# pierluigiferrari/lane_tracker

Hardware: AMD Instinct MI355X
Metric: frames/sec at 1280x720 (end-to-end hot path: undistort+warp+filter_lane_points+sliding_window_search+fit_poly) (higher is better)
Workload: dtype u8; 1 GPU; BASELINE config 3: batch of 256 synthetic lane-like 1280x720 frames per GPU, HBM-resident; warp+filter_lane_points chain + sliding_window_search (26 levels) + fit_poly; bev=1080x1100, parallelism=frames sharded x1, one process per GPU, collective=none (single process), gathered_records_checked=0, streams_per_gpu=4

## Files before the change

include/lane_tracker_amd.h:

```cpp
#ifndef LANE_TRACKER_AMD_H
#define LANE_TRACKER_AMD_H
#include <stddef.h>
#include <stdint.h>

#ifdef __cplusplus
extern "C" {
#endif
#pragma GCC visibility push(default)

#define LT_ABI_VERSION 5

typedef enum lt_status {
    LT_OK = 0,
    LT_ERR_INVALID = -1,
    LT_ERR_HIP = -2,
    LT_ERR_NOMEM = -3,
    LT_ERR_CAPACITY = -4,
    LT_ERR_STATE = -5
} lt_status;

typedef struct lt_ctx lt_ctx;

typedef struct lt_calib {
    int32_t img_w, img_h;
// ... 270 lines not shown
int  lt_calib_warp_table(const lt_calib* calib, int16_t* xy, uint16_t* frac);
int  lt_calib_undistort_table(const lt_calib* calib, int row0, int row1, int16_t* xy, uint16_t* frac);
int  lt_calib_lab_tables(uint16_t* gamma256, uint16_t* cbrt3072, int32_t* coeffs9);
int  lt_calib_ellipse(int k, int32_t* halfwidths , int* taps);

typedef struct lt_gather lt_gather;
int  lt_gather_init(lt_ctx* ctx, int rank, int world, const char* id_path, int timeout_s, lt_gather** out);
int  lt_gather_world(lt_gather* g, int* rank, int* world);
int  lt_gather_reserve(lt_gather* g, int records_per_rank);
int  lt_gather_stage(lt_gather* g, int first_slot, int n, int at);
int  lt_gather_records(lt_gather* g, int n_records, lt_lane_record* out_host);
int  lt_gather_host(lt_gather* g, const void* in, size_t bytes, void* out);
int  lt_gather_barrier(lt_gather* g);
void lt_gather_destroy(lt_gather* g);

int  lt_timer_start(lt_ctx* ctx);
int  lt_timer_stop(lt_ctx* ctx, float* ms);
int  lt_set_stage_timing(lt_ctx* ctx, int enabled);
int  lt_stage_reset(lt_ctx* ctx);
int  lt_stage_ms(lt_ctx* ctx, float* ms, int32_t* launches, int n);
const char* lt_stage_name(int stage);
#define LT_NO_CONTEXT (-2147483647 - 1)
int  lt_last_threshold_path(lt_ctx* ctx);
int  lt_last_tophat_path(lt_ctx* ctx);
int  lt_tophat_split_form(int h, int w, int k, int nbands);
int  lt_last_adaptive_path(lt_ctx* ctx);
int  lt_last_overlay_launches(lt_ctx* ctx);

#pragma GCC visibility pop
#ifdef __cplusplus
}
#endif
#endif
```

lane_tracker_amd/_native.py:

```python
import ctypes as C
import math
import os
import subprocess
import weakref

import numpy as np

_HERE = os.path.dirname(os.path.abspath(__file__))
LIB_PATH = os.environ.get("LANE_TRACKER_AMD_LIB") or os.path.join(_HERE, "liblane_tracker_amd.so")
NUM_STAGES = 12
ABI_VERSION = 5

PLANE_R, PLANE_LAB_B, PLANE_TOPHAT_R, PLANE_TOPHAT_B, PLANE_MERGED, PLANE_MASK = range(6)


class NativeError(RuntimeError):
    pass


class Calib(C.Structure):
    _fields_ = [("img_w", C.c_int32), ("img_h", C.c_int32), ("warp_w", C.c_int32), ("warp_h", C.c_int32),
                ("cam_matrix", C.c_double * 9), ("dist_coeffs", C.c_double * 5), ("M", C.c_double * 9)]


# ... 167 lines not shown
    "lt_calib_lab_tables": (C.c_int, [_P, _P, _P]),
    "lt_calib_ellipse": (C.c_int, [C.c_int, _P, C.POINTER(C.c_int)]),
    "lt_gather_init": (C.c_int, [_P, C.c_int, C.c_int, C.c_char_p, C.c_int, C.POINTER(_P)]),
    "lt_gather_world": (C.c_int, [_P, C.POINTER(C.c_int), C.POINTER(C.c_int)]),
    "lt_gather_reserve": (C.c_int, [_P, C.c_int]),
    "lt_gather_stage": (C.c_int, [_P, C.c_int, C.c_int, C.c_int]),
    "lt_gather_records": (C.c_int, [_P, C.c_int, _P]),
    "lt_gather_host": (C.c_int, [_P, _P, C.c_size_t, _P]),
    "lt_gather_barrier": (C.c_int, [_P]),
    "lt_gather_destroy": (None, [_P]),
    "lt_timer_start": (C.c_int, [_P]),
    "lt_timer_stop": (C.c_int, [_P, C.POINTER(C.c_float)]),
    "lt_set_stage_timing": (C.c_int, [_P, C.c_int]),
    "lt_stage_reset": (C.c_int, [_P]),
    "lt_stage_ms": (C.c_int, [_P, C.POINTER(C.c_float), C.POINTER(C.c_int32), C.c_int]),
    "lt_stage_name": (C.c_char_p, [C.c_int]),
    "lt_device_cache_trim": (C.c_int, [C.c_size_t]),
    "lt_device_cache_stats": (C.c_int, [C.POINTER(C.c_size_t), C.POINTER(C.c_size_t), C.POINTER(C.c_size_t), C.POINTER(C.c_int)]),
    "lt_device_cache_counters": (C.c_int, [C.POINTER(C.c_ulonglong)] * 4),
    "lt_host_memory_stats": (C.c_int, [C.POINTER(C.c_size_t)] * 3),
    "lt_set_download_method": (C.c_int, [_P, C.c_int]),
    "lt_download_stats": (C.c_int, [_P, _P, _P, _P, _P, _P]),
    "lt_last_threshold_path": (C.c_int, [_P]),
    "lt_last_tophat_path": (C.c_int, [_P]),
    "lt_tophat_split_form": (C.c_int, [C.c_int, C.c_int, C.c_int, C.c_int]),
    "lt_last_adaptive_path": (C.c_int, [_P]),
    "lt_set_input_format": (C.c_int, [_P, C.c_int, _P]),
    "lt_get_input_format": (C.c_int, [_P, C.POINTER(C.c_int), _P]),
    "lt_set_input_size": (C.c_int, [_P, C.c_int, C.c_int]),
    "lt_get_input_size": (C.c_int, [_P, C.POINTER(C.c_int), C.POINTER(C.c_int)]),
    "lt_get_input_rows": (C.c_int, [_P, C.POINTER(C.c_int), C.POINTER(C.c_int)]),
    "lt_yuv_to_rgb": (C.c_int, [_P, _P, C.c_int, C.c_int, C.c_int, _P, _P]),
    "lt_bayer_to_rgb": (C.c_int, [_P, _P, C.c_int, C.c_int, C.c_int, _P]),
    "lt_set_raw_lut": (C.c_int, [_P, _P]),
    "lt_get_raw_lut": (C.c_int, [_P, _P, C.POINTER(C.c_int)]),
    "lt_set_raw_lut_wide": (C.c_int, [_P, _P, C.c_size_t]),
    "lt_get_raw_lut_wide": (C.c_int, [_P, _P, C.c_size_t]),
    "lt_raw16_to_rgb": (C.c_int, [_P, _P, C.c_int, C.c_int, C.c_int, _P, _P]),
    "lt_set_raw_color": (C.c_int, [_P, _P, _P, C.c_int]),
    "lt_get_raw_color": (C.c_int, [_P, _P, _P, C.POINTER(C.c_int)]),
    "lt_raw_to_rgb_color": (C.c_int, [_P, _P, C.c_int, C.c_int, C.c_int, _P, C.c_size_t, _P, _P, _P]),
    "lt_set_raw_shading": (C.c_int, [_P, _P, C.c_int, C.c_int, _P, C.c_int]),
    "lt_get_raw_shading": (C.c_int, [_P, _P, C.POINTER(C.c_int), C.POINTER(C.c_int), _P, C.POINTER(C.c_int)]),
    "lt_get_raw_shading_plane": (C.c_int, [_P, _P]),
    "lt_raw_to_rgb_shaded": (C.c_int, [_P, _P, C.c_int, C.c_int, C.c_int, _P, C.c_size_t, _P, _P, _P, C.c_int, C.c_int, _P, _P]),
    "lt_attach_device_frames": (C.c_int, [_P, _P, C.c_int, C.c_int]),
# ... 1290 lines not shown
        coef = (C.c_double * 3)()
        bad = C.c_int(0)
        _check(self.lib.lt_fit_poly2(self._h, ys.ctypes.data, xs.ctypes.data, int(ys.size), self.warp_h, self.warp_w,
                                     coef, C.byref(bad)))
        if bad.value:
            from .lane_tracker import _minimum_norm_parabola
            return _minimum_norm_parabola(ys, xs)
        return np.array(coef[:], np.float64)

    def timer_start(self):
        _check(self.lib.lt_timer_start(self._h))

    def timer_stop(self):
        ms = C.c_float(0)
        _check(self.lib.lt_timer_stop(self._h, C.byref(ms)))
        return ms.value

    def set_stage_timing(self, enabled):
        _check(self.lib.lt_set_stage_timing(self._h, int(bool(enabled))))

    def last_threshold_path(self):
        return int(self.lib.lt_last_threshold_path(self._h))

    def last_tophat_path(self):
        return int(self.lib.lt_last_tophat_path(self._h))

    def last_adaptive_path(self):
        return int(self.lib.lt_last_adaptive_path(self._h))

    def stage_reset(self):
        _check(self.lib.lt_stage_reset(self._h))

    def stage_ms(self):
        ms = (C.c_float * NUM_STAGES)()
        ln = (C.c_int32 * NUM_STAGES)()
        _check(self.lib.lt_stage_ms(self._h, ms, ln, NUM_STAGES))
        return {self.lib.lt_stage_name(i).decode(): (ms[i], ln[i]) for i in range(NUM_STAGES)}


class Gather:

    def __init__(self, ctx, rank, world, id_path, timeout_s=120):
        self._g = None
        self.ctx, self.lib = ctx, ctx.lib
        g = _P()
        _check(self.lib.lt_gather_init(ctx._h, int(rank), int(world), os.fsencode(id_path), int(timeout_s), C.byref(g)))
# ... 49 lines not shown
```

lane_tracker_amd/csrc/lt_api.cpp:

```cpp
#include <algorithm>
#include <atomic>
#include <cmath>
#include <cstdarg>
#include <cstdio>
#include <cstdlib>
#include <chrono>
#include <condition_variable>
#include <cstring>
#include <deque>
#include <map>
#include <memory>
#include <mutex>
#include <string>
#include <thread>
#include <tuple>
#include <vector>
#include <immintrin.h>
#include <sys/mman.h>
#include <unistd.h>

#include <hip/hip_ext.h>

#include "bayer_arith.h"
#include "front_arith.h"
// ... 231 lines not shown

int ensure_band_sums(lt_ctx* c, int nbands) {
    if (nbands <= c->maxbands) return LT_OK;
    int rc = sync_all(c);
    if (rc) return rc;
    dev_free(c->d_band_sums);
    if ((rc = dev_alloc(&c->d_band_sums, (size_t)c->capacity * nbands * c->calib.warp_w))) return rc;
    c->maxbands = nbands;
    return LT_OK;
}

static void preload_kernels(int device, hipStream_t s) {
    static std::mutex m;
    static std::vector<int> done;
    std::lock_guard<std::mutex> g(m);
    if (std::find(done.begin(), done.end(), device) != done.end()) return;
    done.push_back(device);
    TraceScope ts_("lt_create:preload_kernels");
    preload_k_frontend(s);
    preload_k_filter(s);
    preload_k_tophat(s);
    preload_k_threshold(s);
    preload_k_threshold_walk(s);
    preload_k_adaptive_walk(s);
    preload_k_search(s);
    preload_k_overlay(s);
    preload_k_search_viz(s);
    (void)hipStreamSynchronize(s);
    (void)hipGetLastError();
}

int ensure_bev(lt_ctx* c) {
    if (c->d_bev) return LT_OK;
    return dev_alloc(&c->d_bev, (size_t)c->capacity * c->bev_bytes);
}

void mark_masks(lt_ctx* c, int first, int n, int bits_ok, int u8_ok) {
    for (int i = first; i < first + n && i < (int)c->mask_bits_ok.size(); ++i) {
        c->mask_bits_ok[(size_t)i] = (uint8_t)bits_ok;
        c->mask_u8_ok[(size_t)i] = (uint8_t)u8_ok;
    }
}
bool masks_have_bits(const lt_ctx* c, int first, int n) {
    for (int i = first; i < first + n; ++i)
        if (!c->mask_bits_ok[(size_t)i]) return false;
    return true;
}
static int ensure_mask_plane(lt_ctx* c) {
    if (c->masks.d_plane[P_MASK]) return LT_OK;
    const int rc = c->masks.ensure_plane(P_MASK);
    if (rc) return rc;
    HIP_TRY(hipMemsetAsync(c->masks.d_plane[P_MASK], 0, (size_t)c->capacity * c->masks.plane_bytes, c->stream));
    HIP_TRY(hipStreamSynchronize(c->stream));
    return LT_OK;
}
static ChainEnv chain_env(lt_ctx* c) {
    return ChainEnv{&c->se29, &c->se55, c->brute_tophat, c->walk_min_pixels, &c->streams, c->stage_timing ? c : nullptr,
                    &c->last_threshold_path, &c->last_adaptive_path, &c->last_tophat_path};
}
int ensure_u8_masks(lt_ctx* c, int first, int n) {
    bool any = false;
    for (int i = first; i < first + n; ++i) any = any || !c->mask_u8_ok[(size_t)i];
    int rc = ensure_mask_plane(c);
    if (rc) return rc;
    if (!any) return LT_OK;
    if ((rc = sync_all(c))) return rc;
    for (int i = first; i < first + n;) {
        if (c->mask_u8_ok[(size_t)i]) { ++i; continue; }
        int j = i;
        while (j < first + n && !c->mask_u8_ok[(size_t)j]) ++j;
        launch_bits_to_u8(c->stream, slot_bits(c, i, true).bits, slot_mask(c, i),
                          c->calib.warp_h, c->calib.warp_w, c->masks.plane_bytes, c->masks.bits_stride, j - i);
        for (int k = i; k < j; ++k) c->mask_u8_ok[(size_t)k] = 1;
        i = j;
    }
    HIP_TRY(hipGetLastError());
    HIP_TRY(hipStreamSynchronize(c->stream));
    return LT_OK;
}

int make_search_geom(lt_ctx* c, const lt_search_params* p, bool band, SearchGeom& g) {
// ... 2578 lines not shown
}

int lt_timer_start(lt_ctx* c) {
    if (!c) return fail(LT_ERR_INVALID, "null context");
    { int rc = sync_all(c); if (rc) return rc; }
    HIP_TRY(hipEventRecord(c->ev0, c->stream));
    return LT_OK;
}

int lt_timer_stop(lt_ctx* c, float* ms) {
    if (!c || !ms) return fail(LT_ERR_INVALID, "null argument");
    { int rc = sync_all(c); if (rc) return rc; }
    HIP_TRY(hipEventRecord(c->ev1, c->stream));
    HIP_TRY(hipEventSynchronize(c->ev1));
    HIP_TRY(hipEventElapsedTime(ms, c->ev0, c->ev1));
    return LT_OK;
}

int lt_last_threshold_path(lt_ctx* c) {
    if (!c) { (void)fail(LT_ERR_INVALID, "null context"); return LT_NO_CONTEXT; }
    return c->last_threshold_path;
}

int lt_last_tophat_path(lt_ctx* c) {
    if (!c) { (void)fail(LT_ERR_INVALID, "null context"); return LT_NO_CONTEXT; }
    return c->last_tophat_path;
}

int lt_last_overlay_launches(lt_ctx* c) {
    if (!c) { (void)fail(LT_ERR_INVALID, "null context"); return LT_NO_CONTEXT; }
    return c->last_overlay_launches;
}

int lt_tophat_split_form(int h, int w, int k, int nbands) {
    if (h <= 0 || w <= 0 || nbands <= 0) return 0;
    const int band_rows = (h + nbands - 1) / nbands;
    return lt::tophat_split_form(h, w, k, band_rows, (h + band_rows - 1) / band_rows, (w & 3) == 0 && w >= 4) ? 1 : 0;
}

int lt_last_adaptive_path(lt_ctx* c) {
    if (!c) { (void)fail(LT_ERR_INVALID, "null context"); return LT_NO_CONTEXT; }
    return c->last_adaptive_path;
}

int lt_set_stage_timing(lt_ctx* c, int enabled) {
    if (!c) return fail(LT_ERR_INVALID, "null context");
// ... 44 lines not shown
```

lane_tracker_amd/csrc/lt_ctx.h:

```cpp
#pragma once
#include <hip/hip_runtime.h>

#include <algorithm>
#include <functional>
#include <memory>
#include <vector>

#include "lt_internal.h"

namespace lt {

int fail(int code, const char* fmt, ...) __attribute__((format(printf, 2, 3)));

#define HIP_TRY(expr)                                                                               \
    do {                                                                                            \
        hipError_t e_ = (expr);                                                                     \
        if (e_ != hipSuccess) return lt::fail(LT_ERR_HIP, "%s failed: %s", #expr, hipGetErrorString(e_)); \
    } while (0)

enum Stage {
    ST_UNDISTORT = 0, ST_WARP_SPLIT, ST_ERODE_R, ST_TOPHAT_R, ST_ERODE_B, ST_TOPHAT_B, ST_THRESHOLD, ST_MERGE,
    ST_OPEN, ST_SWS_FIT, ST_BAND_FIT, ST_SPLIT_BEV
};

// ... 105 lines not shown
    uint32_t* d_raw_cc = nullptr;
    size_t raw_cc_bytes = 0;
    bool raw_shade_set = false;
    std::vector<uint16_t> raw_mesh;
    int raw_mesh_w = 0, raw_mesh_h = 0;
    lt::RawShade raw_shade = {};
    uint16_t* d_raw_gain = nullptr;
    int src_w = 0, src_h = 0;
    uint8_t* d_src = nullptr;
    size_t src_bytes = 0, src_stride = 0;
    uint32_t* d_rs_xt = nullptr;
    int32_t* d_rs_yt = nullptr;
    std::vector<int32_t> rs_yt;
    lt::SurfEntry* d_surf = nullptr;
    std::vector<lt::SurfEntry> surf;
    std::vector<uint8_t> attached;
    std::vector<uint8_t> drawn;
    uint32_t* d_und = nullptr;
    size_t und_px = 0;
    lt::MaskArena masks;
    lt::VizRing viz;
    int last_threshold_path = -1;
    int last_tophat_path = -1;
    int last_adaptive_path = -1;
    long long walk_min_pixels = 80LL * 1100 * 1080;
    std::vector<uint8_t> mask_bits_ok, mask_u8_ok;
    std::vector<uint8_t> frame_full, annot_full;
    std::vector<uint8_t> front_ok;
    lt_lane_record* d_rec = nullptr;
    double* d_prev = nullptr;
    uint32_t* d_pix = nullptr;
    int32_t* d_cent = nullptr;
    uint32_t* d_band_sums = nullptr;
    lt_search_item* d_items = nullptr;
    lt_search_item* h_items = nullptr;
    int items_cap = 0;
    hipEvent_t items_ev = nullptr;
    int maxpix = 0, maxlev = 0, maxbands = 0;
    bool have_mask = false;
    bool brute_tophat = false;
    int16_t* d_oxy = nullptr;
    uint16_t* d_ofrac = nullptr;
    bool have_overlay = false;
    int16_t* d_spans = nullptr;
    uint8_t* d_annot = nullptr;
    uint8_t* d_strip = nullptr;
// ... 322 lines not shown
            }
        }
        if (c->ev_used + 2 > c->ev_pool.size()) return;
        a = c->ev_pool[c->ev_used++];
        b = c->ev_pool[c->ev_used++];
        (void)hipEventRecord(a, st);
    }
    ~StageScope() {
        if (!a) return;
        (void)hipEventRecord(b, st);
        c->pending.push_back({stage, a, b});
    }
};

int validate_filter(const lt_filter_params* p);
struct ChainEnv {
    const EllipseSE *se29 = nullptr, *se55 = nullptr;
    bool brute_tophat = false;
    long long walk_min_pixels = 0;
    const std::vector<hipStream_t>* streams = nullptr;
    lt_ctx* timing = nullptr;
    int *threshold_path = nullptr, *adaptive_path = nullptr;
    int* tophat_path = nullptr;
};
int run_mask_chain(MaskArena& a, const ChainEnv& env, hipStream_t s, int first, int n, const lt_filter_params* p, int h, int w,
                   int call_frames, bool u8_mask = false);

}
```

lane_tracker_amd/csrc/lt_internal.h:

```cpp
#pragma once
#include <hip/hip_runtime.h>
#include <stdint.h>

#include <vector>

#include <cstdlib>

#include "../../include/lane_tracker_amd.h"
#include "yuv_arith.h"

#ifdef LT_EXPERIMENTS
#define LT_EXP_ENV(name) std::getenv(name)
#else
#define LT_EXP_ENV(name) (static_cast<const char*>(nullptr))
#endif

namespace lt {

struct RemapTable {
    std::vector<int16_t> xy;
    std::vector<uint16_t> frac;
    int rows = 0, cols = 0;
};
void build_warp_table(const lt_calib& c, RemapTable& t);
// ... 90 lines not shown
    const uint16_t* ofrac;
};
static_assert(sizeof(OvTables) == 16, "OvTables: 16 bytes, one scalar load");
struct OvSets {
    const OvTables* sets = nullptr;
    const uint8_t* ids = nullptr;
};
int launch_inplace(hipStream_t s, int layout, const SurfEntry* tab, const SurfEntry* entries, int n, int h, int w, const int rows4[4],
                   InplaceLane l, InplaceText t, YuvCoef kin, const int32_t* rgb2yuv, OvSets per_slot = OvSets());
int launch_draw_to_surfaces(hipStream_t s, int layout, const uint8_t* rgb, size_t rgb_stride, int h, int w, const SurfEntry* entries,
                            int n, const OvTables* sets, const uint8_t* ids, InplaceLane l, InplaceText t, int lane_r0, int lane_r1,
                            const int32_t* coeffs);
void launch_split_bev(hipStream_t s, const uint8_t* bev, size_t bev_stride, int npix, const uint16_t* gamma_tab,
                      const uint16_t* cbrt_tab, const int32_t* coeffs, uint8_t* planeR, uint8_t* planeB,
                      size_t plane_stride, int n);
void launch_undistorted_to_rgb(hipStream_t s, const uint32_t* und, size_t und_px, int first_slot, int nrows, int w, uint8_t* out,
                               int n);

void preload_k_frontend(hipStream_t s);
void preload_k_filter(hipStream_t s);
void preload_k_tophat(hipStream_t s);
void preload_k_threshold(hipStream_t s);
void preload_k_threshold_walk(hipStream_t s);
void preload_k_adaptive_walk(hipStream_t s);
void preload_k_search(hipStream_t s);
void preload_k_overlay(hipStream_t s);

bool launch_overlay_lane_strip(hipStream_t s, const uint8_t* frames, size_t frame_stride, uint8_t* strips, size_t strip_stride,
                               const int16_t* oxy, const uint16_t* ofrac, const int16_t* spans, size_t span_stride_rows, int img_w,
                               int row0, int row1, int bh, int bw, float alpha, int n);
int launch_overlay_lane(hipStream_t s, const uint8_t* frames, uint8_t* out, size_t frame_stride, const int16_t* oxy,
                        const uint16_t* ofrac, const int16_t* spans, size_t span_stride_rows, int img_h, int img_w,
                        int bh, int bw, float alpha, int n, const int* rows4 = nullptr, OvSets per_slot = OvSets());
constexpr int LT_SPAN_ARG_ROWS = 1104;
void launch_store_word(hipStream_t s, unsigned* dev_word, unsigned value);
bool lane_spans_from_regions_available(int bh, int n_rows);
bool launch_lane_spans_from_regions(hipStream_t s, const double* ploty, const double* ploty2, int n_rows, int bh, int bw, int16_t* spans, int n);
bool launch_lane_spans_from_fit(hipStream_t s, const lt_lane_record* rec, const double* prev_sum, int count, const double* ploty,
                                const double* ploty2, int n_rows, int bh, int bw, int16_t* spans);
bool launch_overlay_lane_one(hipStream_t s, const uint8_t* frame, uint8_t* out, const int16_t* oxy, const uint16_t* ofrac,
                             const int16_t* spans_host, int img_h, int img_w, int bh, int bw, float alpha, const int* rows4);
void launch_overlay_text(hipStream_t s, uint8_t* out, size_t frame_stride, int img_h, int img_w, const uint8_t* atlas,
                         const uint8_t* advance, int first_char, int n_glyphs, int gw, int gh, const uint8_t* lines,
                         const int16_t* xpos, int nl, int len, int slot_chars, int y0, int step, int n);
void launch_copy_from_pinned(hipStream_t s, void* dst, const void* src_pinned, size_t bytes);
bool launch_copy_to_pinned(hipStream_t s, void* dst_pinned, const void* src, size_t bytes);
// ... 29 lines not shown
                          unsigned long long* bits_v = nullptr);
void launch_pack_merge(hipStream_t s, const uint8_t* tr, const uint8_t* tb, const uint8_t* labb, const uint8_t* nb,
                       int noise_thresh, int use_noise, unsigned long long* bits, int h, int w, size_t plane_stride,
                       size_t bits_stride, int n);
void launch_open5_bits(hipStream_t s, const unsigned long long* merged, unsigned long long* eroded, uint8_t* mask, int h,
                       int w, size_t plane_stride, size_t bits_stride, int n);
struct MergeInputs {
    unsigned long long* dst = nullptr;
    const unsigned long long* more[3] = {nullptr, nullptr, nullptr};
    int n_more = 0;
    const unsigned long long *and0 = nullptr, *and1 = nullptr;
};
inline int merge_planes(const MergeInputs& in) {
    if (!in.dst || (in.n_more != 0 && in.n_more != 1 && in.n_more != 3)) return 0;
    for (int i = 0; i < 3; ++i)
        if ((in.more[i] != nullptr) != (i < in.n_more)) return 0;
    if ((in.and0 != nullptr) != (in.and1 != nullptr) || (in.and0 && in.n_more != 3)) return 0;
    return in.and0 ? 6 : in.n_more + 1;
}
bool bilateral_walk_supported(int k_r, int C_r, int k_b, int C_b, int h, int w, int pitch, size_t plane_stride);
int launch_bilateral_walk(hipStream_t s, const uint8_t* thr, int k_r, int C_r, const uint8_t* thb, int k_b, int C_b,
                          unsigned long long* merged, unsigned long long* s1, unsigned long long* s2, unsigned long long* s3,
                          int h, int w, int pitch, size_t plane_stride, size_t bits_stride, int n);
void launch_or4_bits(hipStream_t s, const MergeInputs& in, int h, int w, size_t bits_stride, int n);
bool noise_walk_supported(int k_n, int C_n, int h, int w, int pitch, size_t plane_stride);
int launch_noise_walk(hipStream_t s, const uint8_t* braw, int k_n, int C_n, int noise_thresh, unsigned long long* noise_h,
                      unsigned long long* noise_v, int h, int w, int pitch, size_t plane_stride, size_t bits_stride, int n);
bool launch_merge_open5(hipStream_t s, const MergeInputs& in, unsigned long long* opened, int h, int w, size_t bits_stride, int n);
bool launch_or_open5_small(hipStream_t s, const MergeInputs& in, unsigned long long* opened, int h, int w, size_t bits_stride, int n);
void launch_open5_to_bits(hipStream_t s, const unsigned long long* merged, unsigned long long* eroded,
                          unsigned long long* opened, int h, int w, size_t bits_stride, int n);
void launch_bits_to_u8(hipStream_t s, const unsigned long long* bits, uint8_t* out, int h, int w, size_t plane_stride,
                       size_t bits_stride, int n);


struct SearchGeom {
    int h, w;
    int ww, wh, hw;
    int img_height;
    int img_center, y_start, nlevels, limit;
    int nbands;
    int ignore_sides, search_range, def_left, def_right;
    int band_top, band_bottom;
    double mu, bandwidth;
    int maxpix, maxlev;
};
// ... 67 lines not shown
```

lane_tracker_amd/csrc/lt_mask_chain.cpp:

```cpp
#include "lt_ctx.h"

namespace lt {

int validate_filter(const lt_filter_params* p) {
    if (!p) return fail(LT_ERR_INVALID, "null filter params");
    if (p->filter_type != 0 && p->filter_type != 1)
        return fail(LT_ERR_INVALID, "Unexpected filter mode. Expected modes are 'bilateral' or 'neighborhood'.");
    if (p->ksize_r < 1 || p->ksize_b < 1 || (p->mask_noise && p->ksize_noise < 1))
        return fail(LT_ERR_INVALID, "filter sizes must be >= 1");
    if (p->filter_type == 1 && ((p->ksize_r & 1) == 0 || (p->ksize_b & 1) == 0))
        return fail(LT_ERR_INVALID, "'neighborhood' block sizes must be odd (cv2.adaptiveThreshold requirement)");
    if (p->ksize_r > 128 || p->ksize_b > 128 || p->ksize_noise > 128)
        return fail(LT_ERR_INVALID, "filter size too large (max 128)");
    return LT_OK;
}

namespace {

enum TophatForm {
    TH_NONE,
    TH_BRUTE,
    TH_PAIR,
    TH_BATCH
};
// ... 5 lines not shown
    const lt_filter_params* p;
    const int first, n, h, w;
    const bool u8_mask;
    const size_t ps = a.plane_bytes, off = (size_t)first * ps;
    uint8_t *R = a.d_plane[P_R] + off, *B = a.d_plane[P_B] + off, *thR = a.d_plane[P_THR] + off, *thB = a.d_plane[P_THB] + off, *t0 = a.d_plane[P_T0] + off;
    unsigned long long *mbits = a.d_bits_merged + (size_t)first * a.bits_stride, *ebits = a.d_bits_eroded + (size_t)first * a.bits_stride;
    bool walk = false;
    int tophat_path = 0;
    uint8_t *thRd = thR, *thBd = thB, *bpad = nullptr;
    int dpitch = 0;

    int scratch(int idx, uint8_t*& q) {
        const int rc = a.ensure_plane(idx);
        if (!rc) q = a.d_plane[idx] + off;
        return rc;
    }

    int choose_walk(int call_frames) {
        walk = p->filter_type == 0 && !env.brute_tophat && a.walk_planes() && (long long)call_frames * h * w >= env.walk_min_pixels &&
               bilateral_walk_supported(p->ksize_r, p->C_r, p->ksize_b, p->C_b, h, w, a.th_pitch, a.th_pad_bytes) &&
               (!p->mask_noise || noise_walk_supported(p->ksize_noise, p->C_noise, h, w, a.th_pitch, a.th_pad_bytes));
        if (p->filter_type != 0) return LT_OK;
        if (env.threshold_path) *env.threshold_path = walk ? 1 : 0;
        for (int i = first; i < first + n && i < (int)a.th_padded.size(); ++i) a.th_padded[(size_t)i] = walk ? 1 : 0;
        if (!walk) return LT_OK;
        dpitch = a.th_pitch;
        thRd = a.d_th_pad[0] + (size_t)first * a.th_pad_bytes;
        thBd = a.d_th_pad[1] + (size_t)first * a.th_pad_bytes;
        if (p->mask_noise) {
            const int rc = a.ensure_noise_buffers();
            if (rc) return rc;
            bpad = a.d_b_pad + (size_t)first * a.th_pad_bytes;
        }
        return LT_OK;
    }

    int tophat_b(const MorphZone& zone, int* form) {
        if (bpad && launch_morph_runs(s, t0, thBd, B, h, w, 55, true, ps, n, dpitch, a.th_pad_bytes, bpad, zone, form)) return LT_OK;
        launch_morph_runs(s, t0, thBd, B, h, w, 55, true, ps, n, dpitch, a.th_pad_bytes, nullptr, zone, form);
        if (bpad)
            for (int i = 0; i < n; ++i)
                HIP_TRY(hipMemcpy2DAsync(bpad + (size_t)i * a.th_pad_bytes, (size_t)a.th_pitch, B + (size_t)i * ps, (size_t)w, (size_t)w,
                                         (size_t)h, hipMemcpyDeviceToDevice, s));
        return LT_OK;
    }

// ... 31 lines not shown
                zone.stride_dwords = a.zone_stride;
            }
            int f29e = 0, f29d = 0, f55e = 0, f55d = 0;
            { StageScope t(tm, ST_ERODE_R, s);  launch_morph_runs(s, R, t0, nullptr, h, w, 29, false, ps, n, 0, 0, nullptr, zone, &f29e); }
            { StageScope t(tm, ST_TOPHAT_R, s); launch_morph_runs(s, t0, thRd, R, h, w, 29, true, ps, n, dpitch, a.th_pad_bytes, nullptr, zone, &f29d); }
            { StageScope t(tm, ST_ERODE_B, s);  launch_morph_runs(s, B, t0, nullptr, h, w, 55, false, ps, n, 0, 0, nullptr, zone, &f55e); }
            { StageScope t(tm, ST_TOPHAT_B, s); const int rc = tophat_b(zone, &f55d); if (rc) return rc; }
            tophat_path = (f29e && f29d ? 1 : 0) | (f55e && f55d ? 2 : 0);
        }
        if (env.tophat_path && p->filter_type == 0) *env.tophat_path = tophat_path;
        return LT_OK;
    }

    int thresholds(TophatForm form, MergeInputs& in) {
        const size_t bs = a.bits_stride;
        const int noise = p->mask_noise ? 1 : 0;
        in = MergeInputs{};
        in.dst = mbits;
        uint8_t *t1 = nullptr, *t2 = nullptr;
        if (p->filter_type == 0) {
            StageScope t(env.timing, ST_THRESHOLD, s);
            if (walk) {
                unsigned long long *tbits = a.d_bits_tmp + (size_t)first * bs, *ubits = a.d_bits_tmp2 + (size_t)first * bs;
                if (launch_bilateral_walk(s, thRd, p->ksize_r, p->C_r, thBd, p->ksize_b, p->C_b, mbits, ebits, tbits, ubits, h, w, a.th_pitch,
                                          a.th_pad_bytes, bs, n))
                    return fail(LT_ERR_STATE, "the bilateral walk refused parameters its own predicate accepted");
                in.more[0] = ebits, in.more[1] = tbits, in.more[2] = ubits, in.n_more = 3;
                if (!noise) return LT_OK;
                unsigned long long *n1 = a.d_bits_n1 + (size_t)first * bs, *n2 = a.d_bits_n2 + (size_t)first * bs;
                if (launch_noise_walk(s, bpad, p->ksize_noise, p->C_noise, p->noise_thresh, n1, n2, h, w, a.th_pitch, a.th_pad_bytes, bs, n))
                    return fail(LT_ERR_STATE, "the greenery-mask walk refused parameters its own predicate accepted");
                in.and0 = n1; in.and1 = n2;
                return LT_OK;
            }
            if (form == TH_PAIR && !noise &&
                launch_bilateral_bits(s, thR, p->ksize_r, p->C_r, thB, p->ksize_b, p->C_b, B, p->ksize_noise, p->C_noise, p->noise_thresh, 0,
                                      mbits, h, w, ps, bs, n, ebits) == 0) {
                in.more[0] = ebits, in.n_more = 1;
                return LT_OK;
            }
            if (launch_bilateral_bits(s, thR, p->ksize_r, p->C_r, thB, p->ksize_b, p->C_b, B, p->ksize_noise, p->C_noise, p->noise_thresh, noise,
                                      mbits, h, w, ps, bs, n) == 0)
                return LT_OK;
            { int rc = scratch(P_T1, t1); if (!rc) rc = scratch(P_T2, t2); if (rc) return rc; }
            launch_bilateral(s, thR, t1, h, w, p->ksize_r, p->C_r, 0, 255, 0, ps, n);
            launch_bilateral(s, thB, t2, h, w, p->ksize_b, p->C_b, 0, 255, 0, ps, n);
        } else {
            StageScope t(env.timing, ST_THRESHOLD, s);
            const bool box = !noise && launch_adaptive_walk(s, R, p->ksize_r, p->C_r, mbits, B, p->ksize_b, p->C_b, ebits, h, w, ps, bs, n);
// ... 56 lines not shown
```

Measured before the change: 99840 frames/s.

## Compute bilateral threshold box sums with int8 MFMA banded matrix multiplies

Adds a new kernel that evaluates the horizontal and vertical bilateral adaptive-threshold comparisons as banded int8 matrix products on the 32x32x32 MFMA units, packing sign bits into mask words. The walk path now tries this MFMA kernel first and falls back to the sliding-window walk when it is disabled through an environment variable. The aim is to replace the scalar/ALU running-sum walk with matrix-core throughput. The cost is redundant band arithmetic, register pressure from wide prefetch windows, and possible exactness risk in the sign-biased int8 encoding.

```diff
diff --git a/include/lane_tracker_amd.h b/include/lane_tracker_amd.h
--- a/include/lane_tracker_amd.h
+++ b/include/lane_tracker_amd.h
@@ -316,6 +316,7 @@
 const char* lt_stage_name(int stage);
 #define LT_NO_CONTEXT (-2147483647 - 1)
 int  lt_last_threshold_path(lt_ctx* ctx);
+int  lt_last_threshold_form(lt_ctx* ctx);
 int  lt_last_tophat_path(lt_ctx* ctx);
 int  lt_tophat_split_form(int h, int w, int k, int nbands);
 int  lt_last_adaptive_path(lt_ctx* ctx);
diff --git a/lane_tracker_amd/_native.py b/lane_tracker_amd/_native.py
--- a/lane_tracker_amd/_native.py
+++ b/lane_tracker_amd/_native.py
@@ -213,6 +213,7 @@
     "lt_set_download_method": (C.c_int, [_P, C.c_int]),
     "lt_download_stats": (C.c_int, [_P, _P, _P, _P, _P, _P]),
     "lt_last_threshold_path": (C.c_int, [_P]),
+    "lt_last_threshold_form": (C.c_int, [_P]),
     "lt_last_tophat_path": (C.c_int, [_P]),
     "lt_tophat_split_form": (C.c_int, [C.c_int, C.c_int, C.c_int, C.c_int]),
     "lt_last_adaptive_path": (C.c_int, [_P]),
@@ -1549,6 +1550,9 @@
     def last_threshold_path(self):
         return int(self.lib.lt_last_threshold_path(self._h))
 
+    def last_threshold_form(self):
+        return int(self.lib.lt_last_threshold_form(self._h))
+
     def last_tophat_path(self):
         return int(self.lib.lt_last_tophat_path(self._h))
 
diff --git a/lane_tracker_amd/csrc/k_threshold_mma.hip b/lane_tracker_amd/csrc/k_threshold_mma.hip
--- /dev/null
+++ b/lane_tracker_amd/csrc/k_threshold_mma.hip
@@ -0,0 +1,331 @@
+#include <algorithm>
+#include <cstdlib>
+#include <type_traits>
+#include <utility>
+
+#include "lt_internal.h"
+
+namespace lt {
+namespace {
+
+typedef int v4i __attribute__((ext_vector_type(4)));
+typedef int v16i __attribute__((ext_vector_type(16)));
+
+template <class F, int... I>
+__device__ __forceinline__ void static_for(F&& f, std::integer_sequence<int, I...>) {
+    (f(std::integral_constant<int, I>{}), ...);
+}
+
+__device__ __forceinline__ int xcd_contiguous(int id, int n) {
+    const int q = n >> 3, r = n & 7, xcd = id & 7, k = id >> 3;
+    return (xcd < r ? xcd * (q + 1) : r * (q + 1) + (xcd - r) * q) + k;
+}
+
+struct MmaArgs {
+    const uint8_t* src;
+    unsigned long long *out_h, *out_v;
+    int h, w, wpr;
+    int pitch;
+    int C;
+    int hgroups;
+    int vgroups, vsegs, vseg_len;
+    int per_frame;
+    size_t plane_stride, bits_stride;
+};
+
+template <int K>
+struct BandTable {
+    static constexpr int NB = (K + 31) / 32;
+    static constexpr int NOP = NB + 1;
+    uint32_t v[2][2][NOP][64][4];
+};
+constexpr int band_value(int K, int side, int o, int i) {
+    if (i == o) return K;
+    if (side == 0) return (i >= o - K && i <= o - 1) ? -1 : 0;
+    return (i >= o + 1 && i <= o + K) ? -1 : 0;
+}
+template <int K>
+constexpr BandTable<K> make_band() {
+    BandTable<K> t{};
+    constexpr int NB = BandTable<K>::NB;
+    for (int form = 0; form < 2; ++form)
+        for (int side = 0; side < 2; ++side)
+            for (int e = 0; e <= NB; ++e)
+                for (int lane = 0; lane < 64; ++lane) {
+                    const int m = lane & 31, g = lane >> 5, d = side == 0 ? e - NB : e;
+                    const int o = form == 0 ? (m & 3) + 4 * ((m >> 3) & 3) + 16 * ((m >> 2) & 1) : m;
+                    for (int q = 0; q < 4; ++q) {
+                        uint32_t word = 0;
+                        for (int b = 0; b < 4; ++b)
+                            word |= (uint32_t)(band_value(K, side, o, 32 * d + 16 * g + 4 * q + b) & 0xff) << (8 * b);
+                        t.v[form][side][e][lane][q] = word;
+                    }
+                }
+    return t;
+}
+__device__ const BandTable<15> g_band15 = make_band<15>();
+__device__ const BandTable<20> g_band20 = make_band<20>();
+__device__ const BandTable<35> g_band35 = make_band<35>();
+template <int K>
+__device__ __forceinline__ const BandTable<K>& band_table() {
+    if constexpr (K == 15) return g_band15;
+    else if constexpr (K == 20) return g_band20;
+    else return g_band35;
+}
+template <int K, int FORM>
+__device__ __forceinline__ void load_band(v4i (&bl)[BandTable<K>::NOP], v4i (&br)[BandTable<K>::NOP], int lane) {
+    const BandTable<K>& t = band_table<K>();
+#pragma unroll
+    for (int e = 0; e < BandTable<K>::NOP; ++e) {
+        bl[e] = *reinterpret_cast<const v4i*>(&t.v[FORM][0][e][lane][0]);
+        br[e] = *reinterpret_cast<const v4i*>(&t.v[FORM][1][e][lane][0]);
+    }
+}
+
+__device__ __forceinline__ v16i splat16(int c) {
+    v16i v;
+#pragma unroll
+    for (int i = 0; i < 16; ++i) v[i] = c;
+    return v;
+}
+__device__ __forceinline__ v16i mfma(v4i a, v4i b, v16i c) { return __builtin_amdgcn_mfma_i32_32x32x32_i8(a, b, c, 0, 0, 0); }
+__device__ __forceinline__ uint32_t other_half(uint32_t v, int lane) {
+    return (uint32_t)__builtin_amdgcn_ds_bpermute((lane ^ 32) << 2, (int)v);
+}
+
+template <int K>
+struct PrefetchDepth {
+    static constexpr int H = 2, V = 2;
+};
+
+constexpr uint32_t SIGN = 0x80808080u;
+
+template <int K>
+__device__ __forceinline__ void mma_h_task(const MmaArgs& a, int frame, int grp) {
+    constexpr int NB = BandTable<K>::NB, NOP = NB + 1, W = 4 + 2 * NB, D = PrefetchDepth<K>::H;
+    const int lane = threadIdx.x, g = lane >> 5;
+    const int h = a.h, w = a.w;
+    const int row = grp * 32 + (lane & 31);
+    const uint8_t* src = a.src + (size_t)frame * a.plane_stride;
+    const uint32_t lane_off = (uint32_t)__mul24(min(row, h - 1), a.pitch) + 16u * g;
+    unsigned long long* orow = a.out_h + (size_t)frame * a.bits_stride + (size_t)min(row, h - 1) * a.wpr;
+    v4i bl[NOP], br[NOP];
+    load_band<K, 0>(bl, br, lane);
+    const v16i cinit = splat16(-a.C * K - 1);
+
+    const int bmax = (a.pitch >> 5) - 1;
+    auto fetch = [&](int b) -> v4i { return *reinterpret_cast<const v4i*>(src + 32 * min(max(b, 0), bmax) + lane_off); };
+    auto prep = [&](v4i raw, int b) -> v4i {
+        const int col = 32 * b + 16 * g;
+        v4i v;
+#pragma unroll
+        for (int q = 0; q < 4; ++q) v[q] = raw[q] ^ (int)SIGN;
+        if (32 * b < 0 || 32 * b + 32 > w) {
+#pragma unroll
+            for (int q = 0; q < 4; ++q) v[q] = (col + 4 * q >= 0 && col + 4 * q < w) ? v[q] : (int)SIGN;
+        }
+        return v;
+    };
+
+    v4i win[W], pf[D][4];
+#pragma unroll
+    for (int i = 4; i < W; ++i) win[i] = prep(fetch(i - 4 - NB), i - 4 - NB);
+#pragma unroll
+    for (int i = 0; i < 4; ++i) win[i] = win[4];
+#pragma unroll
+    for (int ph = 0; ph < D; ++ph)
+#pragma unroll
+        for (int i = 0; i < 4; ++i) pf[ph][i] = fetch(4 * ph + NB + i);
+    const int trips = (w + 127) >> 7;
+    for (int sb = 0; sb < trips; sb += D) {
+        static_for([&](auto phc) {
+            constexpr int ph = decltype(phc)::value;
+            const int S = sb + ph;
+            if (S < trips) {
+#pragma unroll
+                for (int i = 0; i < 2 * NB; ++i) win[i] = win[i + 4];
+#pragma unroll
+                for (int i = 0; i < 4; ++i) {
+                    win[2 * NB + i] = prep(pf[ph][i], 4 * S + NB + i);
+                    pf[ph][i] = fetch(4 * (S + D) + NB + i);
+                }
+                uint32_t bits[2] = {0u, 0u};
+                static_for([&](auto uc) {
+                    constexpr int u = decltype(uc)::value;
+                    v16i accl = cinit, accr = cinit;
+                    static_for([&](auto ec) {
+                        constexpr int e = decltype(ec)::value;
+                        accl = mfma(bl[e], win[u + e], accl);
+                        accr = mfma(br[e], win[u + e + NB], accr);
+                    }, std::make_integer_sequence<int, NOP>{});
+#pragma unroll
+                    for (int i = 15; i >= 0; --i)
+                        bits[u >> 1] = __builtin_amdgcn_alignbit(bits[u >> 1], (uint32_t)(accl[i] | accr[i]), 31);
+                }, std::make_integer_sequence<int, 4>{});
+                const uint32_t recv = other_half(g ? bits[0] : bits[1], lane);
+                const uint32_t p0 = g ? recv : bits[0], p1 = g ? bits[1] : recv;
+                const uint32_t lo = __builtin_amdgcn_perm(p1, p0, 0x07060302u), hi = __builtin_amdgcn_perm(p1, p0, 0x05040100u);
+                const int word = 2 * S + g;
+                if (row < h && word < a.wpr) orow[word] = ~((unsigned long long)lo | ((unsigned long long)hi << 32));
+            }
+        }, std::make_integer_sequence<int, D>{});
+    }
+}
+
+template <int K>
+__device__ __forceinline__ void mma_v_task(const MmaArgs& a, int frame, int grp, int seg) {
+    constexpr int NB = BandTable<K>::NB, NOP = NB + 1, W = 2 * NB + 1, D = PrefetchDepth<K>::V;
+    const int lane = threadIdx.x, g = lane >> 5;
+    const int h = a.h, w = a.w;
+    const int y0 = seg * a.vseg_len, y1 = min(y0 + a.vseg_len, h);
+    if (y0 >= h) return;
+    const int col = grp * 128 + 4 * (lane & 31);
+    const bool colok = col < w;
+    const uint8_t* src = a.src + (size_t)frame * a.plane_stride;
+    const uint32_t colc = (uint32_t)min(col, w - 4);
+    const uint32_t lane_off = (uint32_t)__mul24(16 * g, a.pitch) + colc;
+    unsigned long long* out = a.out_v + (size_t)frame * a.bits_stride;
+    v4i bl[NOP], br[NOP];
+    load_band<K, 1>(bl, br, lane);
+    const v16i cinit = splat16(-a.C * K - 1);
+
+    struct Raw { uint32_t r[16]; };
+    struct Block { v4i op[4]; };
+    auto fetch = [&](int b) -> Raw {
+        Raw x;
+        if (b >= 0 && 32 * b + 32 <= h) {
+            const uint8_t* base = src + (size_t)(32 * b) * a.pitch;
+#pragma unroll
+            for (int j = 0; j < 16; ++j) x.r[j] = *reinterpret_cast<const uint32_t*>(base + (size_t)j * a.pitch + lane_off);
+        } else {
+#pragma unroll
+            for (int j = 0; j < 16; ++j) {
+                const int r = 32 * b + 16 * g + j;
+                x.r[j] = *reinterpret_cast<const uint32_t*>(src + (uint32_t)__mul24(min(max(r, 0), h - 1), a.pitch) + colc);
+            }
+        }
+        return x;
+    };
+    auto prep = [&](const Raw& x, int b) -> Block {
+        Block o;
+        const bool inside = 32 * b >= 0 && 32 * b + 32 <= h && grp * 128 + 128 <= w;
+#pragma unroll
+        for (int q = 0; q < 4; ++q) {
+            uint32_t r[4];
+#pragma unroll
+            for (int t = 0; t < 4; ++t) {
+                const int y = 32 * b + 16 * g + 4 * q + t;
+                r[t] = x.r[4 * q + t] ^ SIGN;
+                if (!inside) r[t] = (colok && y >= 0 && y < h) ? r[t] : SIGN;
+            }
+            const uint32_t a01 = __builtin_amdgcn_perm(r[1], r[0], 0x05010400u), b01 = __builtin_amdgcn_perm(r[1], r[0], 0x07030602u);
+            const uint32_t a23 = __builtin_amdgcn_perm(r[3], r[2], 0x05010400u), b23 = __builtin_amdgcn_perm(r[3], r[2], 0x07030602u);
+            o.op[0][q] = (int)__builtin_amdgcn_perm(a23, a01, 0x05040100u);
+            o.op[1][q] = (int)__builtin_amdgcn_perm(a23, a01, 0x07060302u);
+            o.op[2][q] = (int)__builtin_amdgcn_perm(b23, b01, 0x05040100u);
+            o.op[3][q] = (int)__builtin_amdgcn_perm(b23, b01, 0x07060302u);
+        }
+        return o;
+    };
+
+    const int t_first = y0 >> 5, t_end = (y1 + 31) >> 5;
+    Block win[W];
+    Raw pf[D];
+#pragma unroll
+    for (int i = 1; i < W; ++i) win[i] = prep(fetch(t_first - NB + i - 1), t_first - NB + i - 1);
+    win[0] = win[1];
+#pragma unroll
+    for (int ph = 0; ph < D; ++ph) pf[ph] = fetch(t_first + NB + ph);
+    for (int tb = t_first; tb < t_end; tb += D) {
+        static_for([&](auto phc) {
+            constexpr int ph = decltype(phc)::value;
+            const int T = tb + ph;
+            if (T < t_end) {
+#pragma unroll
+                for (int i = 0; i + 1 < W; ++i) win[i] = win[i + 1];
+                win[W - 1] = prep(pf[ph], T + NB);
+                pf[ph] = fetch(T + NB + D);
+                uint32_t x = 0u, y = 0u;
+                static_for([&](auto ic) {
+                    constexpr int i = decltype(ic)::value;
+                    v16i accl = cinit, accr = cinit;
+                    static_for([&](auto ec) {
+                        constexpr int e = decltype(ec)::value;
+                        accl = mfma(win[e].op[i], bl[e], accl);
+                        accr = mfma(win[e + NB].op[i], br[e], accr);
+                    }, std::make_integer_sequence<int, NOP>{});
+#pragma unroll
+                    for (int j = 0; j < 16; ++j) {
+                        const uint32_t s = (uint32_t)(accl[j] | accr[j]) >> 31;
+                        const int pos = 16 * ((j >> 2) & 1) + 4 * (j & 3) + i;
+                        if (j < 8) x |= s << pos;
+                        else y |= s << pos;
+                    }
+                }, std::make_integer_sequence<int, 4>{});
+                const uint32_t recv = other_half(g ? x : y, lane);
+                const uint32_t p0 = g ? recv : x, p1 = g ? y : recv;
+                const uint32_t lo = __builtin_amdgcn_perm(p1, p0, 0x05040100u), hi = __builtin_amdgcn_perm(p1, p0, 0x07060302u);
+                const int row = 32 * T + (lane & 31), word = 2 * grp + g;
+                if (row < y1 && word < a.wpr) out[(size_t)row * a.wpr + word] = ~((unsigned long long)lo | ((unsigned long long)hi << 32));
+            }
+        }, std::make_integer_sequence<int, D>{});
+    }
+}
+
+template <int K>
+__global__ __launch_bounds__(64, 2) void k_bilateral_mma_hv(MmaArgs a) {
+    const int b = xcd_contiguous(blockIdx.x, gridDim.x);
+    const int frame = b / a.per_frame, j = b - frame * a.per_frame;
+    const int nh = a.hgroups, nv = a.vgroups * a.vsegs, pairs = min(nh, nv);
+    int v;
+    if (j < 2 * pairs) v = (j & 1) ? (j >> 1) : -1 - (j >> 1);
+    else v = nh > pairs ? -1 - (j - pairs) : j - pairs;
+    if (v < 0) mma_h_task<K>(a, frame, -1 - v);
+    else mma_v_task<K>(a, frame, v / a.vsegs, v % a.vsegs);
+}
+
+template <int K>
+void launch_mma(hipStream_t s, const uint8_t* src, int C, unsigned long long* out_h, unsigned long long* out_v, int h, int w, int pitch,
+                size_t plane_stride, size_t bits_stride, int n) {
+    MmaArgs a;
+    a.src = src;
+    a.out_h = out_h; a.out_v = out_v;
+    a.h = h; a.w = w; a.wpr = (w + 63) / 64;
+    a.pitch = pitch;
+    a.C = C;
+    a.hgroups = (h + 31) / 32;
+    a.vgroups = (w + 127) / 128;
+    a.vsegs = h > 640 ? 2 : 1;
+    a.vseg_len = a.vsegs == 1 ? ((h + 31) & ~31) : (((h + 1) / 2 + 31) & ~31);
+    a.per_frame = a.hgroups + a.vgroups * a.vsegs;
+    a.plane_stride = plane_stride;
+    a.bits_stride = bits_stride;
+    hipLaunchKernelGGL((k_bilateral_mma_hv<K>), dim3((unsigned)(a.per_frame * n)), dim3(64), 0, s, a);
+}
+
+void dispatch_mma(int k, hipStream_t s, const uint8_t* src, int C, unsigned long long* out_h, unsigned long long* out_v, int h, int w,
+                  int pitch, size_t plane_stride, size_t bits_stride, int n) {
+    switch (k) {
+        case 15: launch_mma<15>(s, src, C, out_h, out_v, h, w, pitch, plane_stride, bits_stride, n); break;
+        case 20: launch_mma<20>(s, src, C, out_h, out_v, h, w, pitch, plane_stride, bits_stride, n); break;
+        default: launch_mma<35>(s, src, C, out_h, out_v, h, w, pitch, plane_stride, bits_stride, n); break;
+    }
+}
+
+}
+
+int launch_bilateral_mma(hipStream_t s, const uint8_t* thr, int k_r, int C_r, const uint8_t* thb, int k_b, int C_b,
+                         unsigned long long* merged, unsigned long long* s1, unsigned long long* s2, unsigned long long* s3,
+                         int h, int w, int pitch, size_t plane_stride, size_t bits_stride, int n) {
+    if (n <= 0 || !bilateral_walk_supported(k_r, C_r, k_b, C_b, h, w, pitch, plane_stride)) return -1;
+    static const bool off = [] { const char* e = LT_EXP_ENV("LT_THRESHOLD_MMA"); return e && e[0] == '0'; }();
+    if (off) return 1;
+    dispatch_mma(k_r, s, thr, C_r, merged, s1, h, w, pitch, plane_stride, bits_stride, n);
+    dispatch_mma(k_b, s, thb, C_b, s2, s3, h, w, pitch, plane_stride, bits_stride, n);
+    return 0;
+}
+
+namespace { __global__ void k_preload_k_threshold_mma() {} }
+void preload_k_threshold_mma(hipStream_t s) { hipLaunchKernelGGL(k_preload_k_threshold_mma, dim3(1), dim3(1), 0, s); }
+
+}
diff --git a/lane_tracker_amd/csrc/lt_api.cpp b/lane_tracker_amd/csrc/lt_api.cpp
--- a/lane_tracker_amd/csrc/lt_api.cpp
+++ b/lane_tracker_amd/csrc/lt_api.cpp
@@ -277,6 +277,7 @@
     preload_k_tophat(s);
     preload_k_threshold(s);
     preload_k_threshold_walk(s);
+    preload_k_threshold_mma(s);
     preload_k_adaptive_walk(s);
     preload_k_search(s);
     preload_k_overlay(s);
@@ -311,7 +312,7 @@
 }
 static ChainEnv chain_env(lt_ctx* c) {
     return ChainEnv{&c->se29, &c->se55, c->brute_tophat, c->walk_min_pixels, &c->streams, c->stage_timing ? c : nullptr,
-                    &c->last_threshold_path, &c->last_adaptive_path, &c->last_tophat_path};
+                    &c->last_threshold_path, &c->last_adaptive_path, &c->last_tophat_path, &c->last_threshold_form};
 }
 int ensure_u8_masks(lt_ctx* c, int first, int n) {
     bool any = false;
@@ -2936,6 +2937,11 @@
     return c->last_threshold_path;
 }
 
+int lt_last_threshold_form(lt_ctx* c) {
+    if (!c) { (void)fail(LT_ERR_INVALID, "null context"); return LT_NO_CONTEXT; }
+    return c->last_threshold_form;
+}
+
 int lt_last_tophat_path(lt_ctx* c) {
     if (!c) { (void)fail(LT_ERR_INVALID, "null context"); return LT_NO_CONTEXT; }
     return c->last_tophat_path;
diff --git a/lane_tracker_amd/csrc/lt_ctx.h b/lane_tracker_amd/csrc/lt_ctx.h
--- a/lane_tracker_amd/csrc/lt_ctx.h
+++ b/lane_tracker_amd/csrc/lt_ctx.h
@@ -151,6 +151,7 @@
     lt::VizRing viz;
     int last_threshold_path = -1;
     int last_tophat_path = -1;
+    int last_threshold_form = -1;
     int last_adaptive_path = -1;
     long long walk_min_pixels = 80LL * 1100 * 1080;
     std::vector<uint8_t> mask_bits_ok, mask_u8_ok;
@@ -519,6 +520,7 @@
     lt_ctx* timing = nullptr;
     int *threshold_path = nullptr, *adaptive_path = nullptr;
     int* tophat_path = nullptr;
+    int* threshold_form = nullptr;
 };
 int run_mask_chain(MaskArena& a, const ChainEnv& env, hipStream_t s, int first, int n, const lt_filter_params* p, int h, int w,
                    int call_frames, bool u8_mask = false);
diff --git a/lane_tracker_amd/csrc/lt_internal.h b/lane_tracker_amd/csrc/lt_internal.h
--- a/lane_tracker_amd/csrc/lt_internal.h
+++ b/lane_tracker_amd/csrc/lt_internal.h
@@ -136,6 +136,7 @@
 void preload_k_tophat(hipStream_t s);
 void preload_k_threshold(hipStream_t s);
 void preload_k_threshold_walk(hipStream_t s);
+void preload_k_threshold_mma(hipStream_t s);
 void preload_k_adaptive_walk(hipStream_t s);
 void preload_k_search(hipStream_t s);
 void preload_k_overlay(hipStream_t s);
@@ -211,6 +212,9 @@
 int launch_bilateral_walk(hipStream_t s, const uint8_t* thr, int k_r, int C_r, const uint8_t* thb, int k_b, int C_b,
                           unsigned long long* merged, unsigned long long* s1, unsigned long long* s2, unsigned long long* s3,
                           int h, int w, int pitch, size_t plane_stride, size_t bits_stride, int n);
+int launch_bilateral_mma(hipStream_t s, const uint8_t* thr, int k_r, int C_r, const uint8_t* thb, int k_b, int C_b,
+                         unsigned long long* merged, unsigned long long* s1, unsigned long long* s2, unsigned long long* s3,
+                         int h, int w, int pitch, size_t plane_stride, size_t bits_stride, int n);
 void launch_or4_bits(hipStream_t s, const MergeInputs& in, int h, int w, size_t bits_stride, int n);
 bool noise_walk_supported(int k_n, int C_n, int h, int w, int pitch, size_t plane_stride);
 int launch_noise_walk(hipStream_t s, const uint8_t* braw, int k_n, int C_n, int noise_thresh, unsigned long long* noise_h,
diff --git a/lane_tracker_amd/csrc/lt_mask_chain.cpp b/lane_tracker_amd/csrc/lt_mask_chain.cpp
--- a/lane_tracker_amd/csrc/lt_mask_chain.cpp
+++ b/lane_tracker_amd/csrc/lt_mask_chain.cpp
@@ -51,6 +51,7 @@
                (!p->mask_noise || noise_walk_supported(p->ksize_noise, p->C_noise, h, w, a.th_pitch, a.th_pad_bytes));
         if (p->filter_type != 0) return LT_OK;
         if (env.threshold_path) *env.threshold_path = walk ? 1 : 0;
+        if (env.threshold_form) *env.threshold_form = walk ? 1 : 0;
         for (int i = first; i < first + n && i < (int)a.th_padded.size(); ++i) a.th_padded[(size_t)i] = walk ? 1 : 0;
         if (!walk) return LT_OK;
         dpitch = a.th_pitch;
@@ -128,9 +129,13 @@
             StageScope t(env.timing, ST_THRESHOLD, s);
             if (walk) {
                 unsigned long long *tbits = a.d_bits_tmp + (size_t)first * bs, *ubits = a.d_bits_tmp2 + (size_t)first * bs;
-                if (launch_bilateral_walk(s, thRd, p->ksize_r, p->C_r, thBd, p->ksize_b, p->C_b, mbits, ebits, tbits, ubits, h, w, a.th_pitch,
-                                          a.th_pad_bytes, bs, n))
-                    return fail(LT_ERR_STATE, "the bilateral walk refused parameters its own predicate accepted");
+                int rc = launch_bilateral_mma(s, thRd, p->ksize_r, p->C_r, thBd, p->ksize_b, p->C_b, mbits, ebits, tbits, ubits, h, w, a.th_pitch,
+                                              a.th_pad_bytes, bs, n);
+                if (env.threshold_form) *env.threshold_form = rc == 0 ? 2 : 1;
+                if (rc > 0)
+                    rc = launch_bilateral_walk(s, thRd, p->ksize_r, p->C_r, thBd, p->ksize_b, p->C_b, mbits, ebits, tbits, ubits, h, w, a.th_pitch,
+                                               a.th_pad_bytes, bs, n);
+                if (rc) return fail(LT_ERR_STATE, "the bilateral walk refused parameters its own predicate accepted");
                 in.more[0] = ebits, in.more[1] = tbits, in.more[2] = ubits, in.n_more = 3;
                 if (!noise) return LT_OK;
                 unsigned long long *n1 = a.d_bits_n1 + (size_t)first * bs, *n2 = a.d_bits_n2 + (size_t)first * bs;
```

Result: faster. 106,300 frames/s (median of 6 runs) (+6.5%).
